# tk1363704/CAREL-VAE

Hardware: AMD Instinct MI355X
Metric: clause-pairs/sec (training step) (higher is better)
Workload: dtype bf16

## Files before the change

### carel_vae_amd/csrc/attention.hip

```cpp
#include "carel_hip_internal.h"

namespace carel {

constexpr int HD = 64;
constexpr int NH = 12;
constexpr int HID = NH * HD;
constexpr int QKV_LD = 3 * HID;

__device__ __forceinline__ int f_att(int row) { return (((row >> 1) & 1) << 2) | ((row >> 2) & 3); }
__device__ __forceinline__ int att_off(int row, int chunk) { return row * 128 + ((chunk ^ f_att(row)) << 4); }

__device__ __forceinline__ void stage_att(const bf16_t* __restrict__ g, long ld, int rows, char* img) {
  const int lane = threadIdx.x & 63, wave = __builtin_amdgcn_readfirstlane(threadIdx.x >> 6);
  for (int q = wave; q < (rows >> 3); q += 4) {
    const int r = q * 8 + (lane >> 3);
    const int c = (lane & 7) ^ f_att(r);
    __builtin_amdgcn_global_load_lds(g + (long)r * ld + c * 8, (CAREL_LDS void*)(img + q * 1024), 16, 0, 0);
  }
}

__device__ __forceinline__ bf16x8 frag32_row(const char* img, int r0, int s) {
  const int l = threadIdx.x & 63;
  return *(const bf16x8*)(img + att_off(r0 + (l & 31), 2 * s + (l >> 5)));
}
template <bool PERM>
__device__ __forceinline__ bf16x8 frag32_tr(const char* img, int x0, int kb) {
  const int l = threadIdx.x & 63;
  const int g = l >> 4, hh = g >> 1, qq = (l & 15) >> 2, p = l & 3;
  const int chunk = ((x0 + 16 * (g & 1)) >> 3) + (p >> 1), sub = (p & 1) * 8;
  const int r0 = PERM ? (kb + 4 * hh + qq) : (kb + 8 * hh + qq);
  const int r1 = PERM ? (r0 + 8) : (r0 + 4);
  s16x4 a = __builtin_amdgcn_ds_read_tr16_b64_v4i16((CAREL_LDS s16x4*)(img + att_off(r0, chunk) + sub));
  s16x4 b = __builtin_amdgcn_ds_read_tr16_b64_v4i16((CAREL_LDS s16x4*)(img + att_off(r1, chunk) + sub));
  s16x8 r = {a[0], a[1], a[2], a[3], b[0], b[1], b[2], b[3]};
  return __builtin_bit_cast(bf16x8, r);
}

__device__ __forceinline__ bf16x8 acc_as_operand(const f32x16& x, int s) {
  const uint4 r = {pack2bf(x[8 * s], x[8 * s + 1]), pack2bf(x[8 * s + 2], x[8 * s + 3]), pack2bf(x[8 * s + 4], x[8 * s + 5]), pack2bf(x[8 * s + 6], x[8 * s + 7])};
  return __builtin_bit_cast(bf16x8, r);
}

__device__ __forceinline__ bf16x8 load_frag_global(const bf16_t* p) { return *(const bf16x8*)p; }


__device__ __forceinline__ void store_rows_via_lds(const f32x16 (&acc)[2], float scale, char* slot, bf16_t* grow0, long ld, int row_base, int nrows_live) {
  const int l = threadIdx.x & 63, r = l & 31, hh = l >> 5;
#pragma unroll
  for (int dt = 0; dt < 2; ++dt)
#pragma unroll
    for (int i = 0; i < 4; ++i) {
      const int d = dt * 32 + 8 * i + 4 * hh;
      const int chunk = (d >> 3) ^ ((r >> 1) & 7);
      const uint2 v = {pack2bf(acc[dt][4 * i] * scale, acc[dt][4 * i + 1] * scale), pack2bf(acc[dt][4 * i + 2] * scale, acc[dt][4 * i + 3] * scale)};
      *(uint2*)(slot + r * 128 + chunk * 16 + (d & 4) * 2) = v;
    }
  asm volatile("s_waitcnt lgkmcnt(0)" ::: "memory");
#pragma unroll
  for (int it = 0; it < 4; ++it) {
    const int row = it * 8 + (l >> 3), c = l & 7;
    const uint4 v = *(const uint4*)(slot + row * 128 + ((c ^ ((row >> 1) & 7)) << 4));
    if (row_base + row < nrows_live) *(uint4*)(grow0 + (long)row * ld + c * 8) = v;
  }
  asm volatile("s_waitcnt lgkmcnt(0)" ::: "memory");
}

struct AttnParams {
  const bf16_t* qkv;
  const long* att_mask;
  bf16_t* ctx;
  float* lse;
  const bf16_t* dctx;
  bf16_t* dqkv;
  int B, S;
  Dropout drop;
  const int* cu;
  const float* rel;
  int qlim;
  float* drel;
};

#ifndef CAREL_ATTN_ABLATE
#define CAREL_ATTN_ABLATE 0
#endif
constexpr float MASK_NEG = -3.4028234663852886e38f;
constexpr int ATTN_BWD_LDS = 16384 + 16384 + 32768 + 1024;
constexpr int ATTN_BWD_LDS_REL = ATTN_BWD_LDS + 1024 + 4096;

template <bool REL, bool DROP>
__global__ __launch_bounds__(256, 2) void attn_fwd_kernel(AttnParams p) {
  __shared__ __attribute__((aligned(16))) char smem[2 * 16384 + 512 + (REL ? 1024 : 0)];
  char* kimg = smem;
  char* vimg = smem + 16384;
  float* maskadd = (float*)(smem + 32768);
  float* relb = (float*)(smem + 32768 + 512);
  const int lane = threadIdx.x & 63, wave = threadIdx.x >> 6;
  const int b = blockIdx.x / NH, h = blockIdx.x - b * NH;
  const int S = p.S;
  const long row0 = p.cu ? (long)p.cu[b] : (long)b * S;
  const int len = p.cu ? (p.cu[b + 1] - p.cu[b]) : S;
  const int nkt = (len + 31) >> 5, rows = nkt << 5;
  const bf16_t* qbase = p.qkv + row0 * QKV_LD + h * HD;
  stage_att(qbase + HID, QKV_LD, rows, kimg);
  stage_att(qbase + 2 * HID, QKV_LD, rows, vimg);
  int masked_here = 0;
  for (int k = threadIdx.x; k < rows; k += 256) {
    const float ma = p.cu ? (k < len ? 0.f : MASK_NEG) : ((p.att_mask && p.att_mask[row0 + k] == 0) ? MASK_NEG : 0.f);
    maskadd[k] = ma;
    masked_here |= ma != 0.f;
  }
  if (REL) relb[threadIdx.x] = p.rel[h * 256 + threadIdx.x];
  const int q0 = wave * 32;
  const int hh = lane >> 5;
  bf16x8 qf[4];
  const bool qact = wave < nkt && (p.qlim == 0 || q0 < p.qlim);
  if (qact) {
#pragma unroll
    for (int s = 0; s < 4; ++s) qf[s] = load_frag_global(qbase + (long)(q0 + (lane & 31)) * QKV_LD + 16 * s + 8 * hh);
  }
  asm volatile("s_waitcnt vmcnt(0)" ::: "memory");
  const int any_masked = __syncthreads_or(masked_here);
  if (!qact) return;

  f32x16 x[4];
#pragma unroll
  for (int kt = 0; kt < 4; ++kt) {
#pragma unroll
    for (int r = 0; r < 16; ++r) x[kt][r] = 0.f;
    if (kt < nkt) {
#pragma unroll
      for (int s = 0; s < 4; ++s) x[kt] = mfma32(frag32_row(kimg, kt * 32, s), qf[s], x[kt]);
    }
  }
  constexpr float SC2 = 0.125f * 1.4426950408889634f;
  float m = -INFINITY;
#pragma unroll
  for (int kt = 0; kt < 4; ++kt) {
    if (kt < nkt) {
      const bool tile_masked = p.cu ? (kt == nkt - 1 && (len & 31) != 0) : (any_masked != 0);
      if (tile_masked) {
#pragma unroll
        for (int r = 0; r < 16; ++r) {
          const int key = kt * 32 + acc32_row(r, lane);
          float v = fmaf(x[kt][r], SC2, maskadd[key]);
          if (REL) v = fmaf(relb[127 + key - (q0 + (lane & 31))], 1.4426950408889634f, v);
          x[kt][r] = v;
          m = fmaxf(m, v);
        }
      } else {
#pragma unroll
        for (int r = 0; r < 16; ++r) {
          float v = x[kt][r] * SC2;
          if (REL) v = fmaf(relb[127 + kt * 32 + acc32_row(r, lane) - (q0 + (lane & 31))], 1.4426950408889634f, v);
          x[kt][r] = v;
          m = fmaxf(m, v);
        }
      }
    }
  }
  m = fmaxf(m, __shfl_xor(m, 32, 64));
  float lsum = 0.f;
  const uint32_t ebase = (uint32_t)((((long)b * NH + h) * S + (q0 + (lane & 31))) * S) + (uint32_t)(4 * hh) + p.drop.idx_offset;
#pragma unroll
  for (int kt = 0; kt < 4; ++kt) {
    if (kt < nkt) {
#pragma unroll
      for (int r = 0; r < 16; r += 2) {
        const float e0 = __builtin_amdgcn_exp2f(x[kt][r] - m), e1 = __builtin_amdgcn_exp2f(x[kt][r + 1] - m);
        lsum += e0; lsum += e1;
        float d0 = 1.0f, d1 = 1.0f;
        if constexpr (DROP) {
          const uint32_t hsh = mix32(((ebase + (uint32_t)(kt * 32 + (r & 3) + 8 * (r >> 2))) >> 1) ^ p.drop.key);
          d0 = dropout_pick(p.drop, hsh, 0u); d1 = dropout_pick(p.drop, hsh, 1u);
        }
        x[kt][r] = e0 * d0; x[kt][r + 1] = e1 * d1;
      }
    }
  }
  lsum += __shfl_xor(lsum, 32, 64);
  const bool qlive = q0 + (lane & 31) < len;
  if (hh == 0 && qlive) p.lse[((long)b * NH + h) * S + q0 + (lane & 31)] = (m + __builtin_amdgcn_logf(lsum)) * 0.6931471805599453f;
  const float inv = 1.0f / lsum;
  f32x16 o[2];
#pragma unroll
  for (int dt = 0; dt < 2; ++dt)
#pragma unroll
    for (int r = 0; r < 16; ++r) o[dt][r] = 0.f;
#pragma unroll
  for (int kt = 0; kt < 4; ++kt) {
    if (kt < nkt) {
#pragma unroll
      for (int s = 0; s < 2; ++s) {
        const bf16x8 pf = acc_as_operand(x[kt], s);
#pragma unroll
        for (int dt = 0; dt < 2; ++dt) o[dt] = mfma32(frag32_tr<true>(vimg, dt * 32, kt * 32 + 16 * s), pf, o[dt]);
      }
    }
  }
  bf16_t* crow = p.ctx + (row0 + q0 + (lane & 31)) * HID + h * HD;
  if (qlive) {
#pragma unroll
    for (int dt = 0; dt < 2; ++dt)
#pragma unroll
      for (int i = 0; i < 4; ++i) {
        const int d = dt * 32 + 8 * i + 4 * hh;
        uint2 v = {pack2bf(o[dt][4 * i] * inv, o[dt][4 * i + 1] * inv), pack2bf(o[dt][4 * i + 2] * inv, o[dt][4 * i + 3] * inv)};
        *(uint2*)(crow + d) = v;
      }
  }
}

__device__ __forceinline__ int swz_ds(int k) { return ((k & 3) << 3) | ((k >> 2) & 7); }
__device__ __forceinline__ int ds_off(int k, int q) { return k * 256 + ((((q >> 2) ^ swz_ds(k)) & 31) << 3) + (q & 3) * 2; }

constexpr float LOG2E = 1.4426950408889634f;
template <bool REL, bool DROP>
__global__ __launch_bounds__(256, 2) void attn_bwd_kernel(AttnParams p) {
  extern __shared__ __attribute__((aligned(16))) char smem[];
  char* qimg = smem;
  char* doimg = smem + 16384;
  char* dsimg = smem + 32768;
  float* lse = (float*)(smem + 65536);
  float* delta = lse + 128;
  float* relb = (float*)(smem + ATTN_BWD_LDS);
  float* relg = relb + 256;
  const int lane = threadIdx.x & 63, wave = threadIdx.x >> 6;
  const int b = blockIdx.x / NH, h = blockIdx.x - b * NH;
  const int S = p.S;
  const long row0 = p.cu ? (long)p.cu[b] : (long)b * S;
  const int len = p.cu ? (p.cu[b + 1] - p.cu[b]) : S;
  const int nt = (len + 31) >> 5, rows = nt << 5;
  const int ntq = p.qlim ? min(nt, p.qlim >> 5) : nt;
  const bf16_t* qbase = p.qkv + row0 * QKV_LD + h * HD;
  const bf16_t* dobase = p.dctx + row0 * HID + h * HD;
  const bf16_t* obase = p.ctx + row0 * HID + h * HD;
  stage_att(qbase, QKV_LD, rows, qimg);
  stage_att(dobase, HID, rows, doimg);
  if (REL) {
    relb[threadIdx.x] = p.rel[h * 256 + threadIdx.x];
#pragma unroll
    for (int w = 0; w < 4; ++w) relg[w * 256 + threadIdx.x] = 0.f;
  }
  for (int k = threadIdx.x; k < rows; k += 256) lse[k] = k < len ? fmaxf(p.lse[((long)b * NH + h) * S + k], -1e30f) * LOG2E : INFINITY;
  {
    const int q = threadIdx.x >> 1, half = threadIdx.x & 1;
    float s = 0.f;
    if (q < len) {
      const uint4* a = (const uint4*)(dobase + (long)q * HID + half * 32);
      const uint4* c = (const uint4*)(obase + (long)q * HID + half * 32);
#pragma unroll
      for (int i = 0; i < 4; ++i) {
        const uint4 u = a[i], v = c[i];
        s += bf2f((bf16_t)(u.x & 0xffff)) * bf2f((bf16_t)(v.x & 0xffff)) + bf2f((bf16_t)(u.x >> 16)) * bf2f((bf16_t)(v.x >> 16));
        s += bf2f((bf16_t)(u.y & 0xffff)) * bf2f((bf16_t)(v.y & 0xffff)) + bf2f((bf16_t)(u.y >> 16)) * bf2f((bf16_t)(v.y >> 16));
        s += bf2f((bf16_t)(u.z & 0xffff)) * bf2f((bf16_t)(v.z & 0xffff)) + bf2f((bf16_t)(u.z >> 16)) * bf2f((bf16_t)(v.z >> 16));
        s += bf2f((bf16_t)(u.w & 0xffff)) * bf2f((bf16_t)(v.w & 0xffff)) + bf2f((bf16_t)(u.w >> 16)) * bf2f((bf16_t)(v.w >> 16));
      }
    }
    s += __shfl_xor(s, 1, 64);
    if (q < rows && half == 0) delta[q] = s;
  }
  const int hh = lane >> 5;
  const int kw = wave * 32;
  const bool active = wave < nt;
  bf16x8 kf[4], vf[4];
  if (active) {
#pragma unroll
    for (int s = 0; s < 4; ++s) {
      kf[s] = load_frag_global(qbase + HID + (long)(kw + (lane & 31)) * QKV_LD + 16 * s + 8 * hh);
      vf[s] = load_frag_global(qbase + 2 * HID + (long)(kw + (lane & 31)) * QKV_LD + 16 * s + 8 * hh);
    }
  }
  asm volatile("s_waitcnt vmcnt(0)" ::: "memory");
  __syncthreads();

  f32x16 dk[2], dv[2];
#pragma unroll
  for (int dt = 0; dt < 2; ++dt)
#pragma unroll
    for (int r = 0; r < 16; ++r) { dk[dt][r] = 0.f; dv[dt][r] = 0.f; }
  if (active) {
    const int key = kw + (lane & 31);
    const bool klive = key < len;
    const float madd = p.cu ? (klive ? 0.f : MASK_NEG) : ((p.att_mask && p.att_mask[row0 + key] == 0) ? MASK_NEG : 0.f);
    const float madd2 = madd * LOG2E;
    const uint32_t hbase = (uint32_t)(((long)b * NH + h) * S * S) + (uint32_t)(key & ~1) + (uint32_t)((16 * (lane & 1) + 4 * hh) * S) + p.drop.idx_offset;
    for (int qt = 0; qt < ntq; ++qt) {
      f32x16 sa, dp;
#pragma unroll
      for (int r = 0; r < 16; ++r) { sa[r] = 0.f; dp[r] = 0.f; }
#pragma unroll
      for (int s = 0; s < 4; ++s) {
        sa = mfma32(frag32_row(qimg, qt * 32, s), kf[s], sa);
        dp = mfma32(frag32_row(doimg, qt * 32, s), vf[s], dp);
      }
      uint32_t hown[8], hoth[8];
      const uint32_t odd = (uint32_t)lane & 1u;
      if constexpr (DROP && CAREL_ATTN_ABLATE != 1) {
#pragma unroll
        for (int j = 0; j < 8; ++j) {
          hown[j] = mix32(((hbase + (uint32_t)((qt * 32 + (j & 3) + 8 * (j >> 2)) * S)) >> 1) ^ p.drop.key);
          hoth[j] = (uint32_t)__builtin_amdgcn_update_dpp(0, (int)hown[j], 0xB1, 0xF, 0xF, true);
        }
      }
      f32x16 pd, dsv;
#pragma unroll
      for (int i = 0; i < 4; ++i) {
        const f32x4 l4 = *(const f32x4*)(lse + qt * 32 + 8 * i + 4 * hh);
        const f32x4 d4 = *(const f32x4*)(delta + qt * 32 + 8 * i + 4 * hh);
#pragma unroll
        for (int e = 0; e < 4; ++e) {
          const int r = 4 * i + e;
          float arg = fmaf(sa[r], 0.125f * LOG2E, madd2 - l4[e]);
          if (REL) arg = fmaf(relb[127 + key - (qt * 32 + 8 * i + 4 * hh + e)], LOG2E, arg);
          const float pr = CAREL_ATTN_ABLATE == 3 ? arg : __builtin_amdgcn_exp2f(arg);
          float dm = 1.0f;
          if constexpr (DROP && CAREL_ATTN_ABLATE != 1) dm = dropout_pick(p.drop, ((uint32_t)(r >> 3) == odd) ? hown[r & 7] : hoth[r & 7], odd);
          pd[r] = pr * dm;
          dsv[r] = pr * fmaf(dp[r], dm, -d4[e]);
        }
      }
      if (REL) {
#pragma unroll
        for (int r = 0; r < 16; ++r) {
          float* mine = relg + wave * 256 + 127 + key - (qt * 32 + acc32_row(r, lane));
          if (hh == 0) *mine += dsv[r];
          asm volatile("s_waitcnt lgkmcnt(0)" ::: "memory");
          if (hh == 1) *mine += dsv[r];
          asm volatile("s_waitcnt lgkmcnt(0)" ::: "memory");
        }
      }
#pragma unroll
      for (int i = 0; i < 4; ++i) {
        const int q = qt * 32 + 8 * i + 4 * hh;
        uint2 v = {pack2bf(dsv[4 * i], dsv[4 * i + 1]), pack2bf(dsv[4 * i + 2], dsv[4 * i + 3])};
        *(uint2*)(dsimg + ds_off(key, q)) = v;
      }
#pragma unroll
      for (int s = 0; s < 2; ++s) {
        const bf16x8 pf = acc_as_operand(pd, s), df = acc_as_operand(dsv, s);
#pragma unroll
        for (int dt = 0; dt < 2; ++dt) {
          dv[dt] = mfma32(frag32_tr<true>(doimg, dt * 32, qt * 32 + 16 * s), pf, dv[dt]);
          dk[dt] = mfma32(frag32_tr<true>(qimg, dt * 32, qt * 32 + 16 * s), df, dk[dt]);
        }
      }
    }
  }
  if (CAREL_ATTN_ABLATE == 2) return;
  __syncthreads();
  if (REL && threadIdx.x < 255) {
    const float g = ((relg[threadIdx.x] + relg[256 + threadIdx.x]) + relg[512 + threadIdx.x]) + relg[768 + threadIdx.x];
    p.drel[((long)b * NH + h) * 256 + threadIdx.x] += g;
  }
  stage_att(qbase + HID, QKV_LD, rows, doimg);
  char* slot = qimg + wave * 4096;
  bf16_t* out = p.dqkv + (row0 + kw) * QKV_LD + h * HD;
  if (active && CAREL_ATTN_ABLATE != 4) {
    store_rows_via_lds(dk, 0.125f, slot, out + HID, QKV_LD, kw, len);
    store_rows_via_lds(dv, 1.0f, slot, out + 2 * HID, QKV_LD, kw, len);
  }
  __builtin_amdgcn_sched_barrier(0);
  if (active && !p.cu && CAREL_ATTN_ABLATE != 4) asm volatile("s_waitcnt vmcnt(8)" ::: "memory");
  else asm volatile("s_waitcnt vmcnt(0)" ::: "memory");
  asm volatile("s_waitcnt lgkmcnt(0)" ::: "memory");
  __builtin_amdgcn_s_barrier();
  __builtin_amdgcn_sched_barrier(0);
  if (!active) return;
  f32x16 dq[2];
#pragma unroll
  for (int dt = 0; dt < 2; ++dt)
#pragma unroll
    for (int r = 0; r < 16; ++r) dq[dt][r] = 0.f;
  {
    const int g = lane >> 4, g1 = g & 1, h2 = g >> 1, qq = (lane & 15) >> 2, pp = lane & 3;
    for (int ks = 0; ks < (wave < ntq ? (rows >> 4) : 0); ++ks) {
      const int kr0 = 16 * ks + 8 * h2 + qq, kr1 = kr0 + 4;
      const int qcol = kw + 16 * g1 + 4 * pp;
      s16x4 a = __builtin_amdgcn_ds_read_tr16_b64_v4i16((CAREL_LDS s16x4*)(dsimg + ds_off(kr0, qcol)));
      s16x4 c = __builtin_amdgcn_ds_read_tr16_b64_v4i16((CAREL_LDS s16x4*)(dsimg + ds_off(kr1, qcol)));
      s16x8 bb = {a[0], a[1], a[2], a[3], c[0], c[1], c[2], c[3]};
      const bf16x8 bf = __builtin_bit_cast(bf16x8, bb);
#pragma unroll
      for (int dt = 0; dt < 2; ++dt) dq[dt] = mfma32(frag32_tr<false>(doimg, dt * 32, 16 * ks), bf, dq[dt]);
    }
  }
  if (CAREL_ATTN_ABLATE != 4) store_rows_via_lds(dq, 0.125f, slot, out, QKV_LD, kw, len);
}

}

using namespace carel;

static int attn_prepare(const carel_attn_args* a, AttnParams* p, const char* who, bool bwd) {
  if (!a) return set_error(CAREL_ERR_ARG, "%s: null args", who);
  if (a->heads != NH || a->head_dim != HD) return set_error(CAREL_ERR_SHAPE, "%s: heads/head_dim must be %d/%d", who, NH, HD);
  if (a->seq_len < 32 || a->seq_len > 512 || (a->seq_len & 31)) return set_error(CAREL_ERR_SHAPE, "%s: seq_len must be a multiple of 32 in [32, 512] (got %d)", who, a->seq_len);
  if (a->batch <= 0) return set_error(CAREL_ERR_SHAPE, "%s: batch must be positive", who);
  if (!a->qkv || !a->ctx || !a->lse) return set_error(CAREL_ERR_ARG, "%s: null tensor", who);
  if (bwd && (!a->dctx || !a->dqkv)) return set_error(CAREL_ERR_ARG, "%s: null gradient tensor", who);
  p->qkv = (const bf16_t*)a->qkv; p->att_mask = (const long*)a->attention_mask; p->ctx = (bf16_t*)a->ctx;
  p->lse = (float*)a->lse; p->dctx = (const bf16_t*)a->dctx; p->dqkv = (bf16_t*)a->dqkv;
  p->B = a->batch; p->S = a->seq_len; p->cu = (const int*)a->cu_seqlens;
  p->rel = (const float*)a->rel_bias_dist; p->drel = (float*)a->d_rel_bias_dist;
  if (a->q_rows < 0 || a->q_rows > 128 || (a->q_rows & 31)) return set_error(CAREL_ERR_ARG, "%s: q_rows must be 0, 32, 64 or 96", who);
  p->qlim = a->q_rows >= a->seq_len ? 0 : a->q_rows;
  if (bwd && p->rel && !p->drel) return set_error(CAREL_ERR_ARG, "%s: rel_bias_dist needs d_rel_bias_dist in the backward", who);
  p->drop = make_dropout(a->drop_seed, a->drop_site, a->drop_p, a->drop_idx_offset);
  if (p->drop.thresh != 0 && (a->drop_idx_offset & 1u))
    return set_error(CAREL_ERR_ARG, "%s: drop_idx_offset must be even with dropout on (got %u)", who, a->drop_idx_offset);
  if (p->drop.thresh != 0 && (uint64_t)a->batch * NH * (uint64_t)a->seq_len * a->seq_len + a->drop_idx_offset > 4294967296ull)
    return set_error(CAREL_ERR_SHAPE, "%s: the dropout element index ((b*12 + h)*S + q)*S + k + drop_idx_offset would wrap 32 bits "
                     "(batch %d, seq_len %d, offset %u): split the call", who, a->batch, a->seq_len, a->drop_idx_offset);
  return CAREL_OK;
}

extern "C" int carel_attention_fwd(const carel_attn_args* a, void* stream_) {
  hipStream_t stream = (hipStream_t)stream_;
  AttnParams p;
  int rc = attn_prepare(a, &p, "carel_attention_fwd", false);
  if (rc) return rc;
  if (p.S > 128) return attn_long_fwd(a, stream);
  const bool drop = p.drop.thresh != 0;
  if (p.rel) {
    if (drop) hipLaunchKernelGGL((attn_fwd_kernel<true, true>), dim3(p.B * NH), dim3(256), 0, stream, p);
    else hipLaunchKernelGGL((attn_fwd_kernel<true, false>), dim3(p.B * NH), dim3(256), 0, stream, p);
  } else {
    if (drop) hipLaunchKernelGGL((attn_fwd_kernel<false, true>), dim3(p.B * NH), dim3(256), 0, stream, p);
    else hipLaunchKernelGGL((attn_fwd_kernel<false, false>), dim3(p.B * NH), dim3(256), 0, stream, p);
  }
  return check_launch("attn_fwd_kernel");
}

extern "C" int carel_attention_bwd(const carel_attn_args* a, void* stream_) {
  hipStream_t stream = (hipStream_t)stream_;
  AttnParams p;
  int rc = attn_prepare(a, &p, "carel_attention_bwd", true);
  if (rc) return rc;
  if (p.S > 128) return attn_long_bwd(a, stream);
  static bool attr_set = false;
  if (!attr_set) {
    hipError_t e = hipFuncSetAttribute((const void*)attn_bwd_kernel<false, false>, hipFuncAttributeMaxDynamicSharedMemorySize, ATTN_BWD_LDS);
    if (e == hipSuccess) e = hipFuncSetAttribute((const void*)attn_bwd_kernel<false, true>, hipFuncAttributeMaxDynamicSharedMemorySize, ATTN_BWD_LDS);
    if (e == hipSuccess) e = hipFuncSetAttribute((const void*)attn_bwd_kernel<true, false>, hipFuncAttributeMaxDynamicSharedMemorySize, ATTN_BWD_LDS_REL);
    if (e == hipSuccess) e = hipFuncSetAttribute((const void*)attn_bwd_kernel<true, true>, hipFuncAttributeMaxDynamicSharedMemorySize, ATTN_BWD_LDS_REL);
    if (e != hipSuccess) return set_error(CAREL_ERR_HIP, "carel_attention_bwd: hipFuncSetAttribute: %s", hipGetErrorString(e));
    attr_set = true;
  }
  const bool drop = p.drop.thresh != 0;
  if (p.rel) {
    if (drop) hipLaunchKernelGGL((attn_bwd_kernel<true, true>), dim3(p.B * NH), dim3(256), ATTN_BWD_LDS_REL, stream, p);
    else hipLaunchKernelGGL((attn_bwd_kernel<true, false>), dim3(p.B * NH), dim3(256), ATTN_BWD_LDS_REL, stream, p);
  } else {
    if (drop) hipLaunchKernelGGL((attn_bwd_kernel<false, true>), dim3(p.B * NH), dim3(256), ATTN_BWD_LDS, stream, p);
    else hipLaunchKernelGGL((attn_bwd_kernel<false, false>), dim3(p.B * NH), dim3(256), ATTN_BWD_LDS, stream, p);
  }
  return check_launch("attn_bwd_kernel");
}

namespace carel {
__global__ void relpos_expand_kernel(const float* table, const int* bucket, float* dist) {
  const int h = blockIdx.x, i = threadIdx.x;
  dist[h * 256 + i] = i < 255 ? table[bucket[i] * NH + h] : 0.f;
}
__global__ __launch_bounds__(256) void relpos_reduce_kernel(const float* ddist, int batch, const int* bucket, float* dtable, int accumulate) {
  __shared__ float bydist[256];
  const int h = blockIdx.x, i = threadIdx.x;
  float s = 0.f;
  for (int b = 0; b < batch; ++b) s += ddist[((long)b * NH + h) * 256 + i];
  bydist[i] = s;
  __syncthreads();
  if (i < 32) {
    float t = 0.f;
    for (int d = 0; d < 255; ++d) if (bucket[d] == i) t += bydist[d];
    dtable[i * NH + h] = accumulate ? dtable[i * NH + h] + t : t;
  }
}
}

extern "C" int carel_relpos_expand(const void* table, const void* bucket, void* dist, void* stream) {
  if (!table || !bucket || !dist) return set_error(CAREL_ERR_ARG, "carel_relpos_expand: null tensor");
  hipLaunchKernelGGL(relpos_expand_kernel, dim3(NH), dim3(256), 0, (hipStream_t)stream, (const float*)table, (const int*)bucket, (float*)dist);
  return check_launch("relpos_expand_kernel");
}
extern "C" int carel_relpos_reduce(const void* ddist, int32_t batch, const void* bucket, void* dtable, int32_t accumulate, void* stream) {
  if (!ddist || !bucket || !dtable || batch < 1) return set_error(CAREL_ERR_ARG, "carel_relpos_reduce: null tensor or batch < 1");
  hipLaunchKernelGGL(relpos_reduce_kernel, dim3(NH), dim3(256), 0, (hipStream_t)stream, (const float*)ddist, (int)batch, (const int*)bucket, (float*)dtable, (int)accumulate);
  return check_launch("relpos_reduce_kernel");
}
```

Measured before the change: 8375.

## Shrink attention backward LDS, overlap fwd staging, pack dropout bits

The backward kernel's LDS footprint is cut from 64KB+ to 48KB+. dS is stored in per-qtile slices that reuse the Q image region after a mid-loop barrier, and K for the dQ pass is staged into the freed halves of the Q and dO images. This allows three blocks per CU when relative bias is off. The forward kernel issues mask, rel-bias and Q loads before LDS staging and stages V while QK^T and softmax run. Context stores become 16-byte writes via permlane32_swap. The backward dropout hashes are reduced to a keep bitmask before the DPP exchange, and the dq/dk/dv stores are moved to the end. The new barriers and slice aliasing add complexity and risk of LDS hazards.

```diff
diff --git a/carel_vae_amd/csrc/attention.hip b/carel_vae_amd/csrc/attention.hip
--- a/carel_vae_amd/csrc/attention.hip
+++ b/carel_vae_amd/csrc/attention.hip
@@ -19,13 +19,12 @@
   }
 }
 
-__device__ __forceinline__ bf16x8 frag32_row(const char* img, int r0, int s) {
-  const int l = threadIdx.x & 63;
+__device__ __forceinline__ bf16x8 frag32_row(const char* img, int r0, int s, int l) {
   return *(const bf16x8*)(img + att_off(r0 + (l & 31), 2 * s + (l >> 5)));
 }
+__device__ __forceinline__ bf16x8 frag32_row(const char* img, int r0, int s) { return frag32_row(img, r0, s, threadIdx.x & 63); }
 template <bool PERM>
-__device__ __forceinline__ bf16x8 frag32_tr(const char* img, int x0, int kb) {
-  const int l = threadIdx.x & 63;
+__device__ __forceinline__ bf16x8 frag32_tr(const char* img, int x0, int kb, int l) {
   const int g = l >> 4, hh = g >> 1, qq = (l & 15) >> 2, p = l & 3;
   const int chunk = ((x0 + 16 * (g & 1)) >> 3) + (p >> 1), sub = (p & 1) * 8;
   const int r0 = PERM ? (kb + 4 * hh + qq) : (kb + 8 * hh + qq);
@@ -35,6 +34,9 @@
   s16x8 r = {a[0], a[1], a[2], a[3], b[0], b[1], b[2], b[3]};
   return __builtin_bit_cast(bf16x8, r);
 }
+
+template <bool PERM>
+__device__ __forceinline__ bf16x8 frag32_tr(const char* img, int x0, int kb) { return frag32_tr<PERM>(img, x0, kb, threadIdx.x & 63); }
 
 __device__ __forceinline__ bf16x8 acc_as_operand(const f32x16& x, int s) {
   const uint4 r = {pack2bf(x[8 * s], x[8 * s + 1]), pack2bf(x[8 * s + 2], x[8 * s + 3]), pack2bf(x[8 * s + 4], x[8 * s + 5]), pack2bf(x[8 * s + 6], x[8 * s + 7])};
@@ -84,7 +86,7 @@
 #define CAREL_ATTN_ABLATE 0
 #endif
 constexpr float MASK_NEG = -3.4028234663852886e38f;
-constexpr int ATTN_BWD_LDS = 16384 + 16384 + 32768 + 1024;
+constexpr int ATTN_BWD_LDS = 16384 + 16384 + 16384 + 1024;
 constexpr int ATTN_BWD_LDS_REL = ATTN_BWD_LDS + 1024 + 4096;
 
 template <bool REL, bool DROP>
@@ -101,15 +103,11 @@
   const int len = p.cu ? (p.cu[b + 1] - p.cu[b]) : S;
   const int nkt = (len + 31) >> 5, rows = nkt << 5;
   const bf16_t* qbase = p.qkv + row0 * QKV_LD + h * HD;
-  stage_att(qbase + HID, QKV_LD, rows, kimg);
-  stage_att(qbase + 2 * HID, QKV_LD, rows, vimg);
-  int masked_here = 0;
-  for (int k = threadIdx.x; k < rows; k += 256) {
-    const float ma = p.cu ? (k < len ? 0.f : MASK_NEG) : ((p.att_mask && p.att_mask[row0 + k] == 0) ? MASK_NEG : 0.f);
-    maskadd[k] = ma;
-    masked_here |= ma != 0.f;
-  }
-  if (REL) relb[threadIdx.x] = p.rel[h * 256 + threadIdx.x];
+  const int mk = threadIdx.x;
+  long mask_in = 1;
+  if (mk < rows && !p.cu && p.att_mask) mask_in = p.att_mask[row0 + mk];
+  float rel_in = 0.f;
+  if (REL) rel_in = p.rel[h * 256 + threadIdx.x];
   const int q0 = wave * 32;
   const int hh = lane >> 5;
   bf16x8 qf[4];
@@ -118,77 +116,96 @@
 #pragma unroll
     for (int s = 0; s < 4; ++s) qf[s] = load_frag_global(qbase + (long)(q0 + (lane & 31)) * QKV_LD + 16 * s + 8 * hh);
   }
+  stage_att(qbase + HID, QKV_LD, rows, kimg);
+  asm volatile("" : "+v"(mask_in), "+v"(rel_in) :: "memory");
+  int masked_here = 0;
+  if (mk < rows) {
+    const float ma = p.cu ? (mk < len ? 0.f : MASK_NEG) : (mask_in == 0 ? MASK_NEG : 0.f);
+    maskadd[mk] = ma;
+    masked_here = ma != 0.f;
+  }
+  if (REL) relb[threadIdx.x] = rel_in;
   asm volatile("s_waitcnt vmcnt(0)" ::: "memory");
   const int any_masked = __syncthreads_or(masked_here);
+
+  f32x16 x[4];
+  float inv = 0.f;
+  const bool qlive = q0 + (lane & 31) < len;
+  if (qact) {
+#pragma unroll
+    for (int kt = 0; kt < 4; ++kt) {
+#pragma unroll
+      for (int r = 0; r < 16; ++r) x[kt][r] = 0.f;
+      if (kt < nkt) {
+#pragma unroll
+        for (int s = 0; s < 4; ++s) x[kt] = mfma32(frag32_row(kimg, kt * 32, s), qf[s], x[kt]);
+      }
+    }
+  }
+  stage_att(qbase + 2 * HID, QKV_LD, rows, vimg);
+  if (qact) {
+    constexpr float SC2 = 0.125f * 1.4426950408889634f;
+    float m = -INFINITY;
+#pragma unroll
+    for (int kt = 0; kt < 4; ++kt) {
+      if (kt < nkt) {
+        const bool tile_masked = p.cu ? (kt == nkt - 1 && (len & 31) != 0) : (any_masked != 0);
+        if (tile_masked) {
+#pragma unroll
+          for (int r = 0; r < 16; ++r) {
+            const int key = kt * 32 + acc32_row(r, lane);
+            float v = fmaf(x[kt][r], SC2, maskadd[key]);
+            if (REL) v = fmaf(relb[127 + key - (q0 + (lane & 31))], 1.4426950408889634f, v);
+            x[kt][r] = v;
+            m = fmaxf(m, v);
+          }
+        } else {
+#pragma unroll
+          for (int r = 0; r < 16; ++r) {
+            float v = x[kt][r] * SC2;
+            if (REL) v = fmaf(relb[127 + kt * 32 + acc32_row(r, lane) - (q0 + (lane & 31))], 1.4426950408889634f, v);
+            x[kt][r] = v;
+            m = fmaxf(m, v);
+          }
+        }
+      }
+    }
+    m = fmaxf(m, __shfl_xor(m, 32, 64));
+    float lsum = 0.f;
+    const uint32_t ebase = (uint32_t)((((long)b * NH + h) * S + (q0 + (lane & 31))) * S) + (uint32_t)(4 * hh) + p.drop.idx_offset;
+#pragma unroll
+    for (int kt = 0; kt < 4; ++kt) {
+      if (kt < nkt) {
+#pragma unroll
+        for (int r = 0; r < 16; r += 2) {
+          const float e0 = __builtin_amdgcn_exp2f(x[kt][r] - m), e1 = __builtin_amdgcn_exp2f(x[kt][r + 1] - m);
+          lsum += e0; lsum += e1;
+          float d0 = 1.0f, d1 = 1.0f;
+          if constexpr (DROP) {
+            const uint32_t hsh = mix32(((ebase + (uint32_t)(kt * 32 + (r & 3) + 8 * (r >> 2))) >> 1) ^ p.drop.key);
+            d0 = dropout_pick(p.drop, hsh, 0u); d1 = dropout_pick(p.drop, hsh, 1u);
+          }
+          x[kt][r] = e0 * d0; x[kt][r + 1] = e1 * d1;
+        }
+      }
+    }
+    lsum += __shfl_xor(lsum, 32, 64);
+    if (hh == 0 && qlive) p.lse[((long)b * NH + h) * S + q0 + (lane & 31)] = (m + __builtin_amdgcn_logf(lsum)) * 0.6931471805599453f;
+    inv = 1.0f / lsum;
+  }
+  __builtin_amdgcn_sched_barrier(0);
+  asm volatile("s_waitcnt vmcnt(0)" ::: "memory");
+  __builtin_amdgcn_s_barrier();
+  __builtin_amdgcn_sched_barrier(0);
   if (!qact) return;
-
-  f32x16 x[4];
-#pragma unroll
-  for (int kt = 0; kt < 4; ++kt) {
-#pragma unroll
-    for (int r = 0; r < 16; ++r) x[kt][r] = 0.f;
-    if (kt < nkt) {
-#pragma unroll
-      for (int s = 0; s < 4; ++s) x[kt] = mfma32(frag32_row(kimg, kt * 32, s), qf[s], x[kt]);
-    }
-  }
-  constexpr float SC2 = 0.125f * 1.4426950408889634f;
-  float m = -INFINITY;
+  f32x16 o[2];
+#pragma unroll
+  for (int dt = 0; dt < 2; ++dt)
+#pragma unroll
+    for (int r = 0; r < 16; ++r) o[dt][r] = 0.f;
 #pragma unroll
   for (int kt = 0; kt < 4; ++kt) {
     if (kt < nkt) {
-      const bool tile_masked = p.cu ? (kt == nkt - 1 && (len & 31) != 0) : (any_masked != 0);
-      if (tile_masked) {
-#pragma unroll
-        for (int r = 0; r < 16; ++r) {
-          const int key = kt * 32 + acc32_row(r, lane);
-          float v = fmaf(x[kt][r], SC2, maskadd[key]);
-          if (REL) v = fmaf(relb[127 + key - (q0 + (lane & 31))], 1.4426950408889634f, v);
-          x[kt][r] = v;
-          m = fmaxf(m, v);
-        }
-      } else {
-#pragma unroll
-        for (int r = 0; r < 16; ++r) {
-          float v = x[kt][r] * SC2;
-          if (REL) v = fmaf(relb[127 + kt * 32 + acc32_row(r, lane) - (q0 + (lane & 31))], 1.4426950408889634f, v);
-          x[kt][r] = v;
-          m = fmaxf(m, v);
-        }
-      }
-    }
-  }
-  m = fmaxf(m, __shfl_xor(m, 32, 64));
-  float lsum = 0.f;
-  const uint32_t ebase = (uint32_t)((((long)b * NH + h) * S + (q0 + (lane & 31))) * S) + (uint32_t)(4 * hh) + p.drop.idx_offset;
-#pragma unroll
-  for (int kt = 0; kt < 4; ++kt) {
-    if (kt < nkt) {
-#pragma unroll
-      for (int r = 0; r < 16; r += 2) {
-        const float e0 = __builtin_amdgcn_exp2f(x[kt][r] - m), e1 = __builtin_amdgcn_exp2f(x[kt][r + 1] - m);
-        lsum += e0; lsum += e1;
-        float d0 = 1.0f, d1 = 1.0f;
-        if constexpr (DROP) {
-          const uint32_t hsh = mix32(((ebase + (uint32_t)(kt * 32 + (r & 3) + 8 * (r >> 2))) >> 1) ^ p.drop.key);
-          d0 = dropout_pick(p.drop, hsh, 0u); d1 = dropout_pick(p.drop, hsh, 1u);
-        }
-        x[kt][r] = e0 * d0; x[kt][r + 1] = e1 * d1;
-      }
-    }
-  }
-  lsum += __shfl_xor(lsum, 32, 64);
-  const bool qlive = q0 + (lane & 31) < len;
-  if (hh == 0 && qlive) p.lse[((long)b * NH + h) * S + q0 + (lane & 31)] = (m + __builtin_amdgcn_logf(lsum)) * 0.6931471805599453f;
-  const float inv = 1.0f / lsum;
-  f32x16 o[2];
-#pragma unroll
-  for (int dt = 0; dt < 2; ++dt)
-#pragma unroll
-    for (int r = 0; r < 16; ++r) o[dt][r] = 0.f;
-#pragma unroll
-  for (int kt = 0; kt < 4; ++kt) {
-    if (kt < nkt) {
 #pragma unroll
       for (int s = 0; s < 2; ++s) {
         const bf16x8 pf = acc_as_operand(x[kt], s);
@@ -197,30 +214,30 @@
       }
     }
   }
-  bf16_t* crow = p.ctx + (row0 + q0 + (lane & 31)) * HID + h * HD;
-  if (qlive) {
-#pragma unroll
-    for (int dt = 0; dt < 2; ++dt)
-#pragma unroll
-      for (int i = 0; i < 4; ++i) {
-        const int d = dt * 32 + 8 * i + 4 * hh;
-        uint2 v = {pack2bf(o[dt][4 * i] * inv, o[dt][4 * i + 1] * inv), pack2bf(o[dt][4 * i + 2] * inv, o[dt][4 * i + 3] * inv)};
-        *(uint2*)(crow + d) = v;
-      }
-  }
-}
-
-__device__ __forceinline__ int swz_ds(int k) { return ((k & 3) << 3) | ((k >> 2) & 7); }
-__device__ __forceinline__ int ds_off(int k, int q) { return k * 256 + ((((q >> 2) ^ swz_ds(k)) & 31) << 3) + (q & 3) * 2; }
+  bf16_t* crow = p.ctx + (row0 + q0 + (lane & 31)) * HID + h * HD + 8 * hh;
+#pragma unroll
+  for (int dt = 0; dt < 2; ++dt)
+#pragma unroll
+    for (int i = 0; i < 4; i += 2) {
+      uint2 va = {pack2bf(o[dt][4 * i] * inv, o[dt][4 * i + 1] * inv), pack2bf(o[dt][4 * i + 2] * inv, o[dt][4 * i + 3] * inv)};
+      uint2 vb = {pack2bf(o[dt][4 * i + 4] * inv, o[dt][4 * i + 5] * inv), pack2bf(o[dt][4 * i + 6] * inv, o[dt][4 * i + 7] * inv)};
+      const auto sx = __builtin_amdgcn_permlane32_swap(va.x, vb.x, false, false);
+      const auto sy = __builtin_amdgcn_permlane32_swap(va.y, vb.y, false, false);
+      const uint4 v = {sx[0], sy[0], sx[1], sy[1]};
+      if (qlive) *(uint4*)(crow + dt * 32 + 8 * i) = v;
+    }
+}
+
+__device__ __forceinline__ int ds_off(int k, int q) { return k * 64 + ((((q >> 2) ^ (k >> 2)) & 7) << 3) + (q & 3) * 2; }
 
 constexpr float LOG2E = 1.4426950408889634f;
 template <bool REL, bool DROP>
-__global__ __launch_bounds__(256, 2) void attn_bwd_kernel(AttnParams p) {
+__global__ __launch_bounds__(256, REL ? 2 : 3) void attn_bwd_kernel(AttnParams p) {
   extern __shared__ __attribute__((aligned(16))) char smem[];
   char* qimg = smem;
   char* doimg = smem + 16384;
-  char* dsimg = smem + 32768;
-  float* lse = (float*)(smem + 65536);
+  auto ds_slice = [&](int t) { return smem + (t < 2 ? 32768 + t * 8192 : (t - 2) * 16384); };
+  float* lse = (float*)(smem + 49152);
   float* delta = lse + 128;
   float* relb = (float*)(smem + ATTN_BWD_LDS);
   float* relg = relb + 256;
@@ -234,31 +251,18 @@
   const bf16_t* qbase = p.qkv + row0 * QKV_LD + h * HD;
   const bf16_t* dobase = p.dctx + row0 * HID + h * HD;
   const bf16_t* obase = p.ctx + row0 * HID + h * HD;
-  stage_att(qbase, QKV_LD, rows, qimg);
-  stage_att(dobase, HID, rows, doimg);
-  if (REL) {
-    relb[threadIdx.x] = p.rel[h * 256 + threadIdx.x];
-#pragma unroll
-    for (int w = 0; w < 4; ++w) relg[w * 256 + threadIdx.x] = 0.f;
-  }
-  for (int k = threadIdx.x; k < rows; k += 256) lse[k] = k < len ? fmaxf(p.lse[((long)b * NH + h) * S + k], -1e30f) * LOG2E : INFINITY;
-  {
-    const int q = threadIdx.x >> 1, half = threadIdx.x & 1;
-    float s = 0.f;
-    if (q < len) {
-      const uint4* a = (const uint4*)(dobase + (long)q * HID + half * 32);
-      const uint4* c = (const uint4*)(obase + (long)q * HID + half * 32);
-#pragma unroll
-      for (int i = 0; i < 4; ++i) {
-        const uint4 u = a[i], v = c[i];
-        s += bf2f((bf16_t)(u.x & 0xffff)) * bf2f((bf16_t)(v.x & 0xffff)) + bf2f((bf16_t)(u.x >> 16)) * bf2f((bf16_t)(v.x >> 16));
-        s += bf2f((bf16_t)(u.y & 0xffff)) * bf2f((bf16_t)(v.y & 0xffff)) + bf2f((bf16_t)(u.y >> 16)) * bf2f((bf16_t)(v.y >> 16));
-        s += bf2f((bf16_t)(u.z & 0xffff)) * bf2f((bf16_t)(v.z & 0xffff)) + bf2f((bf16_t)(u.z >> 16)) * bf2f((bf16_t)(v.z >> 16));
-        s += bf2f((bf16_t)(u.w & 0xffff)) * bf2f((bf16_t)(v.w & 0xffff)) + bf2f((bf16_t)(u.w >> 16)) * bf2f((bf16_t)(v.w >> 16));
-      }
-    }
-    s += __shfl_xor(s, 1, 64);
-    if (q < rows && half == 0) delta[q] = s;
+  const int lk = threadIdx.x;
+  float lse_in = 0.f;
+  if (lk < len) lse_in = p.lse[((long)b * NH + h) * S + lk];
+  float rel_in = 0.f;
+  if (REL) rel_in = p.rel[h * 256 + threadIdx.x];
+  const int dq_row = threadIdx.x >> 1, half = threadIdx.x & 1;
+  uint4 d_do[4], d_o[4];
+  if (dq_row < len) {
+    const uint4* a = (const uint4*)(dobase + (long)dq_row * HID + half * 32);
+    const uint4* c = (const uint4*)(obase + (long)dq_row * HID + half * 32);
+#pragma unroll
+    for (int i = 0; i < 4; ++i) { d_do[i] = a[i]; d_o[i] = c[i]; }
   }
   const int hh = lane >> 5;
   const int kw = wave * 32;
@@ -271,6 +275,33 @@
       vf[s] = load_frag_global(qbase + 2 * HID + (long)(kw + (lane & 31)) * QKV_LD + 16 * s + 8 * hh);
     }
   }
+  long kmask_in = 1;
+  if (active && !p.cu && p.att_mask) kmask_in = p.att_mask[row0 + kw + (lane & 31)];
+  stage_att(qbase, QKV_LD, rows, qimg);
+  stage_att(dobase, HID, rows, doimg);
+  asm volatile("" : "+v"(lse_in), "+v"(rel_in), "+v"(kmask_in) :: "memory");
+  if (REL) {
+    relb[threadIdx.x] = rel_in;
+#pragma unroll
+    for (int w = 0; w < 4; ++w) relg[w * 256 + threadIdx.x] = 0.f;
+  }
+  if (lk < rows) lse[lk] = lk < len ? fmaxf(lse_in, -1e30f) * LOG2E : INFINITY;
+  {
+    const int q = dq_row;
+    float s = 0.f;
+    if (q < len) {
+#pragma unroll
+      for (int i = 0; i < 4; ++i) {
+        const uint4 u = d_do[i], v = d_o[i];
+        s += bf2f((bf16_t)(u.x & 0xffff)) * bf2f((bf16_t)(v.x & 0xffff)) + bf2f((bf16_t)(u.x >> 16)) * bf2f((bf16_t)(v.x >> 16));
+        s += bf2f((bf16_t)(u.y & 0xffff)) * bf2f((bf16_t)(v.y & 0xffff)) + bf2f((bf16_t)(u.y >> 16)) * bf2f((bf16_t)(v.y >> 16));
+        s += bf2f((bf16_t)(u.z & 0xffff)) * bf2f((bf16_t)(v.z & 0xffff)) + bf2f((bf16_t)(u.z >> 16)) * bf2f((bf16_t)(v.z >> 16));
+        s += bf2f((bf16_t)(u.w & 0xffff)) * bf2f((bf16_t)(v.w & 0xffff)) + bf2f((bf16_t)(u.w >> 16)) * bf2f((bf16_t)(v.w >> 16));
+      }
+    }
+    s += __shfl_xor(s, 1, 64);
+    if (q < rows && half == 0) delta[q] = s;
+  }
   asm volatile("s_waitcnt vmcnt(0)" ::: "memory");
   __syncthreads();
 
@@ -279,35 +310,47 @@
   for (int dt = 0; dt < 2; ++dt)
 #pragma unroll
     for (int r = 0; r < 16; ++r) { dk[dt][r] = 0.f; dv[dt][r] = 0.f; }
-  if (active) {
+  {
     const int key = kw + (lane & 31);
     const bool klive = key < len;
-    const float madd = p.cu ? (klive ? 0.f : MASK_NEG) : ((p.att_mask && p.att_mask[row0 + key] == 0) ? MASK_NEG : 0.f);
+    const float madd = p.cu ? (klive ? 0.f : MASK_NEG) : (kmask_in == 0 ? MASK_NEG : 0.f);
     const float madd2 = madd * LOG2E;
     const uint32_t hbase = (uint32_t)(((long)b * NH + h) * S * S) + (uint32_t)(key & ~1) + (uint32_t)((16 * (lane & 1) + 4 * hh) * S) + p.drop.idx_offset;
     for (int qt = 0; qt < ntq; ++qt) {
+      if (qt == 2) __syncthreads();
+      if (!active) continue;
+      char* dsimg = ds_slice(qt);
+      int l1 = lane, l2 = lane, l3 = lane;
+      asm volatile("" : "+v"(l1));
       f32x16 sa, dp;
 #pragma unroll
       for (int r = 0; r < 16; ++r) { sa[r] = 0.f; dp[r] = 0.f; }
 #pragma unroll
-      for (int s = 0; s < 4; ++s) {
-        sa = mfma32(frag32_row(qimg, qt * 32, s), kf[s], sa);
-        dp = mfma32(frag32_row(doimg, qt * 32, s), vf[s], dp);
-      }
-      uint32_t hown[8], hoth[8];
-      const uint32_t odd = (uint32_t)lane & 1u;
+      for (int s = 0; s < 4; ++s) sa = mfma32(frag32_row(qimg, qt * 32, s, l1), kf[s], sa);
+      asm volatile("" : "+v"(sa) :: "memory");
+#pragma unroll
+      for (int s = 0; s < 4; ++s) dp = mfma32(frag32_row(doimg, qt * 32, s, l1), vf[s], dp);
+      uint32_t keep = 0;
       if constexpr (DROP && CAREL_ATTN_ABLATE != 1) {
+        const uint32_t odd = (uint32_t)lane & 1u, t16 = p.drop.thresh >> 16;
+        uint32_t mine = 0, theirs = 0;
 #pragma unroll
         for (int j = 0; j < 8; ++j) {
-          hown[j] = mix32(((hbase + (uint32_t)((qt * 32 + (j & 3) + 8 * (j >> 2)) * S)) >> 1) ^ p.drop.key);
-          hoth[j] = (uint32_t)__builtin_amdgcn_update_dpp(0, (int)hown[j], 0xB1, 0xF, 0xF, true);
+          const uint32_t hsh = mix32(((hbase + (uint32_t)((qt * 32 + (j & 3) + 8 * (j >> 2)) * S)) >> 1) ^ p.drop.key);
+          const uint32_t lo = hsh & 0xffffu, hi = hsh >> 16;
+          mine |= (uint32_t)((odd ? hi : lo) >= t16) << j;
+          theirs |= (uint32_t)((odd ? lo : hi) >= t16) << j;
         }
+        theirs = (uint32_t)__builtin_amdgcn_update_dpp(0, (int)theirs, 0xB1, 0xF, 0xF, true);
+        keep = odd ? (theirs | (mine << 8)) : (mine | (theirs << 8));
       }
       f32x16 pd, dsv;
+      asm volatile("" : "+v"(l2));
+      const int hh2 = l2 >> 5;
 #pragma unroll
       for (int i = 0; i < 4; ++i) {
-        const f32x4 l4 = *(const f32x4*)(lse + qt * 32 + 8 * i + 4 * hh);
-        const f32x4 d4 = *(const f32x4*)(delta + qt * 32 + 8 * i + 4 * hh);
+        const f32x4 l4 = *(const f32x4*)(lse + qt * 32 + 8 * i + 4 * hh2);
+        const f32x4 d4 = *(const f32x4*)(delta + qt * 32 + 8 * i + 4 * hh2);
 #pragma unroll
         for (int e = 0; e < 4; ++e) {
           const int r = 4 * i + e;
@@ -315,7 +358,7 @@
           if (REL) arg = fmaf(relb[127 + key - (qt * 32 + 8 * i + 4 * hh + e)], LOG2E, arg);
           const float pr = CAREL_ATTN_ABLATE == 3 ? arg : __builtin_amdgcn_exp2f(arg);
           float dm = 1.0f;
-          if constexpr (DROP && CAREL_ATTN_ABLATE != 1) dm = dropout_pick(p.drop, ((uint32_t)(r >> 3) == odd) ? hown[r & 7] : hoth[r & 7], odd);
+          if constexpr (DROP && CAREL_ATTN_ABLATE != 1) dm = ((keep >> r) & 1u) ? p.drop.scale : 0.0f;
           pd[r] = pr * dm;
           dsv[r] = pr * fmaf(dp[r], dm, -d4[e]);
         }
@@ -332,17 +375,18 @@
       }
 #pragma unroll
       for (int i = 0; i < 4; ++i) {
-        const int q = qt * 32 + 8 * i + 4 * hh;
+        const int q = 8 * i + 4 * hh2;
         uint2 v = {pack2bf(dsv[4 * i], dsv[4 * i + 1]), pack2bf(dsv[4 * i + 2], dsv[4 * i + 3])};
-        *(uint2*)(dsimg + ds_off(key, q)) = v;
-      }
+        *(uint2*)(dsimg + ds_off(kw + (l2 & 31), q)) = v;
+      }
+      asm volatile("" : "+v"(l3));
 #pragma unroll
       for (int s = 0; s < 2; ++s) {
         const bf16x8 pf = acc_as_operand(pd, s), df = acc_as_operand(dsv, s);
 #pragma unroll
         for (int dt = 0; dt < 2; ++dt) {
-          dv[dt] = mfma32(frag32_tr<true>(doimg, dt * 32, qt * 32 + 16 * s), pf, dv[dt]);
-          dk[dt] = mfma32(frag32_tr<true>(qimg, dt * 32, qt * 32 + 16 * s), df, dk[dt]);
+          dv[dt] = mfma32(frag32_tr<true>(doimg, dt * 32, qt * 32 + 16 * s, l3), pf, dv[dt]);
+          dk[dt] = mfma32(frag32_tr<true>(qimg, dt * 32, qt * 32 + 16 * s, l3), df, dk[dt]);
         }
       }
     }
@@ -353,39 +397,40 @@
     const float g = ((relg[threadIdx.x] + relg[256 + threadIdx.x]) + relg[512 + threadIdx.x]) + relg[768 + threadIdx.x];
     p.drel[((long)b * NH + h) * 256 + threadIdx.x] += g;
   }
-  stage_att(qbase + HID, QKV_LD, rows, doimg);
-  char* slot = qimg + wave * 4096;
-  bf16_t* out = p.dqkv + (row0 + kw) * QKV_LD + h * HD;
-  if (active && CAREL_ATTN_ABLATE != 4) {
-    store_rows_via_lds(dk, 0.125f, slot, out + HID, QKV_LD, kw, len);
-    store_rows_via_lds(dv, 1.0f, slot, out + 2 * HID, QKV_LD, kw, len);
-  }
-  __builtin_amdgcn_sched_barrier(0);
-  if (active && !p.cu && CAREL_ATTN_ABLATE != 4) asm volatile("s_waitcnt vmcnt(8)" ::: "memory");
-  else asm volatile("s_waitcnt vmcnt(0)" ::: "memory");
-  asm volatile("s_waitcnt lgkmcnt(0)" ::: "memory");
-  __builtin_amdgcn_s_barrier();
-  __builtin_amdgcn_sched_barrier(0);
+  char* const k_lo = qimg + 8192;
+  char* const k_hi = doimg + 8192 - 64 * 128;
+  stage_att(qbase + HID, QKV_LD, min(rows, 64), k_lo);
+  if (rows > 64) stage_att(qbase + HID + 64L * QKV_LD, QKV_LD, rows - 64, doimg + 8192);
+  asm volatile("s_waitcnt vmcnt(0)" ::: "memory");
+  __syncthreads();
   if (!active) return;
   f32x16 dq[2];
 #pragma unroll
   for (int dt = 0; dt < 2; ++dt)
 #pragma unroll
     for (int r = 0; r < 16; ++r) dq[dt][r] = 0.f;
+  char* const mine = ds_slice(wave);
   {
     const int g = lane >> 4, g1 = g & 1, h2 = g >> 1, qq = (lane & 15) >> 2, pp = lane & 3;
     for (int ks = 0; ks < (wave < ntq ? (rows >> 4) : 0); ++ks) {
       const int kr0 = 16 * ks + 8 * h2 + qq, kr1 = kr0 + 4;
-      const int qcol = kw + 16 * g1 + 4 * pp;
-      s16x4 a = __builtin_amdgcn_ds_read_tr16_b64_v4i16((CAREL_LDS s16x4*)(dsimg + ds_off(kr0, qcol)));
-      s16x4 c = __builtin_amdgcn_ds_read_tr16_b64_v4i16((CAREL_LDS s16x4*)(dsimg + ds_off(kr1, qcol)));
+      const int qcol = 16 * g1 + 4 * pp;
+      s16x4 a = __builtin_amdgcn_ds_read_tr16_b64_v4i16((CAREL_LDS s16x4*)(mine + ds_off(kr0, qcol)));
+      s16x4 c = __builtin_amdgcn_ds_read_tr16_b64_v4i16((CAREL_LDS s16x4*)(mine + ds_off(kr1, qcol)));
       s16x8 bb = {a[0], a[1], a[2], a[3], c[0], c[1], c[2], c[3]};
       const bf16x8 bf = __builtin_bit_cast(bf16x8, bb);
-#pragma unroll
-      for (int dt = 0; dt < 2; ++dt) dq[dt] = mfma32(frag32_tr<false>(doimg, dt * 32, 16 * ks), bf, dq[dt]);
-    }
-  }
-  if (CAREL_ATTN_ABLATE != 4) store_rows_via_lds(dq, 0.125f, slot, out, QKV_LD, kw, len);
+      const char* kimg = ks < 4 ? k_lo : k_hi;
+#pragma unroll
+      for (int dt = 0; dt < 2; ++dt) dq[dt] = mfma32(frag32_tr<false>(kimg, dt * 32, 16 * ks), bf, dq[dt]);
+    }
+  }
+  if (CAREL_ATTN_ABLATE != 4) {
+    asm volatile("s_waitcnt lgkmcnt(0)" ::: "memory");
+    bf16_t* out = p.dqkv + (row0 + kw) * QKV_LD + h * HD;
+    store_rows_via_lds(dq, 0.125f, mine, out, QKV_LD, kw, len);
+    store_rows_via_lds(dk, 0.125f, mine, out + HID, QKV_LD, kw, len);
+    store_rows_via_lds(dv, 1.0f, mine, out + 2 * HID, QKV_LD, kw, len);
+  }
 }
 
 }
```

New measurement: 8470 (median of 6 runs). +1.1%, better.
